# mryndzionek/composable-sdr

Hardware: AMD Instinct MI355X
Metric: MS/s CF32 throughput, 256-ch PFB+FM pipeline (higher is better)
Workload: dtype f32; 1 GPU; cfg3: 256-ch firpfbch(m=7,As=80)+dcBlocker+freqdem(kf=0.3) on synthetic CF32, AGC off (-a 0), 262144 frames/step (512 MiB in, 256 MiB out), HBM-resident; channels=256, demod=fm, mix=False, route=fused-256|k_tile256<FM>, preheat_steps=10999, collective=none, rccl_ranks=1

## Files before the change

composable_sdr_amd/csrc/fused.h:

```cpp
#pragma once
#include "csdr_internal.h"

namespace csdr {

struct FusedConfig {
    uint32_t M, p, C, c0, max_nf;
    uint32_t G = 1;
    bool dc_block; DcParams dc;
    bool fm; float fm_ref;
    bool mix;
    const float *taps;
    uint32_t d_theta;
    uint32_t cus = 256;
};

struct FusedCall {
    const float2 *d_in;
    void *d_out;
    uint32_t nf;
    uint32_t theta0;
    bool indep = false;
    hipEvent_t ev_tail = nullptr;
    bool tile_major = false;
};
// ... 25 lines not shown
    std::vector<float2> premix_table() const;
    virtual int reset_state(hipStream_t s) = 0;
    virtual int run(const FusedCall &call, void *out, hipStream_t s, KernelTimer *timer) = 0;
};

template <class Plan> int make_plan(const FusedConfig &cfg, ChainPlan **out)
{
    Plan *p = new Plan(cfg);
    if (int r = p->init()) { delete p; return r; }
    *out = p;
    return 0;
}

bool plan256_supported(uint32_t M, uint32_t p);
int  plan256_create(const FusedConfig &cfg, ChainPlan **out);
bool plan64_supported(uint32_t M, uint32_t p);
int  plan64_create(const FusedConfig &cfg, ChainPlan **out);
bool plan1024_supported(uint32_t M, uint32_t p);
int  plan1024_create(const FusedConfig &cfg, ChainPlan **out);
bool plan4096_supported(uint32_t M, uint32_t p);
int  plan4096_create(const FusedConfig &cfg, ChainPlan **out);

int  run256_v2_launch(const void *run_args, bool fm, unsigned G, unsigned nruns, hipStream_t s);
int  run256_v2_blocks_per_cu(bool fm);
int  run256_dcfix_launch(const void *run_args, bool fm, unsigned nruns, const float2 *Rt, hipStream_t s);
int  run256_v3_launch(const void *run_args, bool fm, unsigned nruns, hipStream_t s);


struct Run64v2Host {
    const float2 *x; float2 *out;
    const float *taps; const float2 *tw, *wpre;
    const float2 *uhist_in; float2 *uhist_out; const float2 *vend_in; float2 *vend_out;
    float2 *cpre = nullptr; const float2 *rt = nullptr;
    uint32_t nf, nruns, parity0;
    uint32_t G = 1, g = 0;
    bool tile_major = false;
    bool dc_block;
    double beta;
};
constexpr int RUN64_DCFIX_F = 448;
uint32_t run64_v2_runs(uint32_t nf, uint32_t cus);
void dc_state_response(const FusedConfig &cfg, const float2 *wpre, uint32_t f0, uint32_t nfr, uint32_t k0, float2 *rt);
int run64_v2_launch(const Run64v2Host &h, hipStream_t s, KernelTimer *timer);

struct Run1024v2Host {
    const float2 *x; void *out;
    const float4 *taps_q;
// ... 37 lines not shown
```

composable_sdr_amd/csrc/fused_v2_common.h:

```cpp
#pragma once
#include "fused_common.h"

namespace csdr {
namespace {

typedef float v4f __attribute__((ext_vector_type(4)));
#ifndef V2_DMA_AUX
#define V2_DMA_AUX ""
#endif
#ifndef V2_DMA_AUX_STREAM
#define V2_DMA_AUX_STREAM V2_DMA_AUX
#endif

__device__ __forceinline__ void bar()
{
    asm volatile("s_waitcnt lgkmcnt(0)\n\ts_barrier" ::: "memory");
}
__device__ __forceinline__ float opaque_v(float x) { asm volatile("" : "+v"(x)); return x; }

__device__ __forceinline__ unsigned dma_offset(int tid)
{
    const int wave = tid >> 6, lane = tid & 63;
    const int slot = 64 * wave + lane, q = slot >> 3, i = (slot & 7) ^ ((q >> 1) & 7);
    return (unsigned)(8 * q + i) * 16u;
// ... 2 lines not shown
{
    const int wave = tid >> 6, lane = tid & 63;
    const int slot = 64 * wave + lane, q = slot >> 3, i = (slot & 7) ^ (q & 7);
    return (unsigned)(8 * q + i) * 16u;
}
template <bool STREAM = false, unsigned IT_STEP = 4096u>
__device__ __forceinline__ void dma_tile(const float4 *__restrict__ tile_base, unsigned goff, unsigned lds_wave)
{
    asm volatile("" : "+s"(lds_wave));
#pragma unroll
    for (int it = 0; it < 8; it++) {
        const unsigned dst = lds_wave + IT_STEP * (unsigned)it;
        const float4 *src = tile_base + 256 * it;
        unsigned keep;
        if (STREAM)
            asm volatile("s_mov_b32 %0, m0\n\ts_mov_b32 m0, %2\n\ts_nop 4\n\tglobal_load_lds_dwordx4 %1, %3" V2_DMA_AUX_STREAM "\n\ts_mov_b32 m0, %0"
                         : "=&s"(keep) : "v"(goff), "s"(dst), "s"(src) : "memory");
        else
            asm volatile("s_mov_b32 %0, m0\n\ts_mov_b32 m0, %2\n\ts_nop 4\n\tglobal_load_lds_dwordx4 %1, %3" V2_DMA_AUX "\n\ts_mov_b32 m0, %0"
                         : "=&s"(keep) : "v"(goff), "s"(dst), "s"(src) : "memory");
    }
}

__device__ __forceinline__ void dma_piece(const float4 *__restrict__ tile_base, unsigned goff, unsigned lds_wave, const int it)
{
    asm volatile("" : "+s"(lds_wave));
    const unsigned dst = lds_wave + 4096u * (unsigned)it;
    const float4 *src = tile_base + 256 * it;
    unsigned keep;
    asm volatile("s_mov_b32 %0, m0\n\ts_mov_b32 m0, %2\n\ts_nop 4\n\tglobal_load_lds_dwordx4 %1, %3" V2_DMA_AUX "\n\ts_mov_b32 m0, %0"
                 : "=&s"(keep) : "v"(goff), "s"(dst), "s"(src) : "memory");
}

struct FmK { float tiny, ref, hp, pi; };
__device__ __forceinline__ float fm_sample(float2 rp, float2 r, const FmK &k)
{
    const float re = fmaf(rp.x, r.x, rp.y * r.y);
    const float im = fmaf(rp.x, r.y, -(rp.y * r.x));
    const float mx = fmaxf(fmaxf(fabsf(re), fabsf(im)), k.tiny);
    const float mn = fminf(fabsf(re), fabsf(im));
    const float a = mn * __builtin_amdgcn_rcpf(mx);
    const float z = a * a;
    float p = -4.054457881e-03f;
    p = fmaf(p, z, 2.186254039e-02f);
    p = fmaf(p, z, -5.591168255e-02f);
    p = fmaf(p, z, 9.642146528e-02f);
    p = fmaf(p, z, -1.390860826e-01f);
    p = fmaf(p, z, 1.994656026e-01f);
    p = fmaf(p, z, -3.332985938e-01f);
    p = fmaf(p, z, 9.999993443e-01f);
// ... 92 lines not shown
```

composable_sdr_amd/csrc/kernels_fused.hip:

```cpp
#include "fused_common.h"
#include <cstring>

namespace csdr {

namespace {

#define STAMP(i) do { if (A.trace && tid == 0) A.trace[(size_t)b * 16 + (i)] = __builtin_amdgcn_s_memtime(); } while (0)

template <bool FM>
__global__ __launch_bounds__(256) void k_tile256(TileArgs A)
{
    __shared__ __attribute__((aligned(16))) float2 R[LDS_F2];
    __shared__ float2 tw_s[M256];
    __shared__ float2 Tt[2][16];
    __shared__ float2 carry_s[2];
    __shared__ unsigned tile_s;

    const int tid = threadIdx.x;
    if (tid == 0) tile_s = atomicAdd(A.ticket, 1u);
    tw_s[tid] = A.tw[tid];
    __syncthreads();
    const unsigned b = tile_s;
    if (b >= A.nb) return;
    STAMP(0);
// ... 425 lines not shown
    CSDR_HIP(hipMemcpy(d_wpre, wpre.data(), sizeof(float2) * 2 * cfg.M, hipMemcpyHostToDevice));
    if (nowu) {
        std::vector<float2> rt((size_t)2 * DCFIX_F * 4);
        dc_state_response(cfg, wpre.data(), 15u, (uint32_t)DCFIX_F, 126u, rt.data());
        CSDR_HIP(hipMemcpy(d_rt, rt.data(), sizeof(float2) * rt.size(), hipMemcpyHostToDevice));
    }
    CSDR_HIP(hipMemset(d_status, 0, sizeof(unsigned)));
    CSDR_HIP(hipMemset(d_yflag, 0, sizeof(unsigned) * max_nb));
    CSDR_HIP(hipMemset(d_agg, 0, sizeof(u64) * 2 * max_nb));

    TileArgs &A = proto;
    A = TileArgs{};
    A.taps = d_taps; A.tw = d_tw; A.wpre = d_wpre;
    A.ticket = d_ticket; A.agg = d_agg; A.ylast = d_ylast; A.yflag = d_yflag; A.status = d_status;
    A.c0 = cfg.c0; A.C = cfg.C; A.fm_ref = cfg.fm_ref; A.trace = d_trace;
    const double beta = cfg.dc_block ? (double)cfg.dc.beta : 0.0;
    A.alpha = cfg.dc_block ? (float)(1.0 - beta) : 0.0f;
    A.beta = (float)beta;
    for (int k = 0; k < LOOKBACK + 2; k++) A.wtile[k] = (float)std::pow(beta, 4096.0 * k);
    for (int k = 0; k < 16; k++) A.b16[k] = (float)std::pow(beta, 16.0 * k);
    for (int k = 0; k < 17; k++) A.b256[k] = (float)std::pow(beta, 256.0 * k);
    for (int k = 0; k < 16; k++) A.bj[k] = (float)std::pow(beta, (double)k);
    if (const char *e = diag_env("CSDR_CUS")) { if (atoi(e) > 0 && (uint32_t)atoi(e) < cus) cus = (uint32_t)atoi(e); }
    resident_wgs_v2 = (uint32_t)(cus * run256_v2_blocks_per_cu(cfg.fm));
    if (const char *e = diag_env("CSDR_RESIDENT_WGS")) resident_wgs_v2 = (uint32_t)atol(e);
#ifdef CSDR_WITH_RUN256_V3
    if (const char *e = diag_env("CSDR_RUN_V3")) use_v3 = atoi(e) != 0;
#endif
    if (const char *e = diag_env("CSDR_RUN_WEIGHTS")) {
        int k = 0;
        for (const char *q = e; *q && k < 8; k++) { slot_weight[k] = (float)atof(q); q = strchr(q, ','); if (!q) break; q++; }
    }
    return 0;
}

int FusedPlan::reset_state(hipStream_t s)
{
    for (int i = 0; i < 2; i++) {
        CSDR_HIP(hipMemsetAsync(d_yhist[i], 0, sizeof(float2) * 13 * cfg.M, s));
        CSDR_HIP(hipMemsetAsync(d_vend[i], 0, sizeof(float2), s));
        CSDR_HIP(hipMemsetAsync(d_rp[i], 0, sizeof(float2) * (cfg.G > 1 ? cfg.M : cfg.C), s));
    }
    CSDR_HIP(hipMemsetAsync(d_tail[0], 0, sizeof(float4) * 2048 * (WU + 1), s));
    tail_w = 0; tail_valid = true;
    return 0;
}

// ... 22 lines not shown
    A.rp_in = d_rp[cur];       A.rp_out = d_rp[cur ^ 1];
    A.out_stride = nf; A.out_t0 = 0;
    if (call.tile_major) A.out_stride = NB;
    A.parity0 = (uint32_t)(frames_done & 1);
    const uint32_t nb_full = nf / NB;
    const bool shard = c.G > 1;
    if (shard && (uint64_t)c.C * nf * (c.fm ? 4u : 8u) >= (1ull << 32)) { set_error("fused: interleaved shard output of %u frames exceeds 4 GiB", nf); return -1; }
    const bool whole_band = c.G == 1 && c.c0 == 0 && c.C == c.M;
    if ((nb_full >= run_min_tiles && whole_band) || shard) {
        const bool v2 = true;
        const bool v3 = !shard && use_v3;
        kernel = v3 ? (c.fm ? "k_run256v3<FM>" : "k_run256v3<CF32>") : (c.fm ? "k_run256v2<FM>" : "k_run256v2<CF32>");
        if (shard) kernel += "/G" + std::to_string(c.G);
        RunArgs RA{};
        A.nf = nb_full * NB; A.nb = nb_full;
        RA.t = A; RA.pk = phase_consts(c.fm_ref);
        uint32_t nruns = v3 ? cus : resident_wgs_v2;
        if (v3) { if (const char *e = diag_env("CSDR_V3_RUNS")) nruns = (uint32_t)atol(e); }
        if (nruns > A.nb / 8) nruns = A.nb / 8;
        if (nruns < 1) nruns = 1;
        RA.nruns = nruns;
        static const float v2_weight_cf[8] = {1.2f, 0.8f, 1.f, 1.f, 1.f, 1.f, 1.f, 1.f};
        static const float v2_weight_fm[8] = {1.24f, 0.76f, 1.f, 1.f, 1.f, 1.f, 1.f, 1.f};
        const float *v2_weight = c.fm ? v2_weight_fm : v2_weight_cf;
        static const float equal_weight[8] = {1.f, 1.f, 1.f, 1.f, 1.f, 1.f, 1.f, 1.f};
        static const bool pd_equal = diag_env("CSDR_PD_EQUAL") != nullptr;
        RA.split = make_split(A.nb, nruns, cus, (call.indep && pd_equal) ? equal_weight : ((v2 && !diag_env("CSDR_RUN_WEIGHTS")) ? v2_weight : slot_weight));
        { const char *e = diag_env("CSDR_PRIO_ROT"); RA.prio_div = e ? (atoi(e) ? cus : 0u) : (v2 ? 0u : cus); }
        { const char *e = diag_env("CSDR_TRACE"); RA.trace_light = (e && atoi(e) == 2) ? 1u : 0u; }
        { const char *e = diag_env("CSDR_WU"); RA.wu = e ? (uint32_t)atoi(e) : (uint32_t)WU; }
        { const char *e = diag_env("CSDR_WU_ROT"); RA.wu_rot = e ? (uint32_t)atoi(e) : 0u; }
        RA.pair_align = (v2 && (c.fm || diag_env("CSDR_PAIR_ALIGN_CF"))) ? 1u : 0u;
        { const char *e = diag_env("CSDR_WU_BATCH6"); RA.wu_batch6 = e ? (uint32_t)atoi(e) : 1u; }
        RA.l2beta = c.dc_block ? (float)std::log2((double)c.dc.beta) : -1000.0f;
        RA.tile_step = call.tile_major ? c.C * 128u : (uint32_t)NB * (c.fm ? 4u : 8u);
        const bool whole = nf == nb_full * NB;
        RA.indep = call.indep ? 1u : 0u;
        RA.nowu = (nowu && !shard && !v3 && !RA.indep && nruns >= 2 && nruns <= 2048) ? 1u : 0u;
        RA.cpre = d_cpre; RA.side = d_side;
        RA.prev_tail = d_tail[tail_w];
        if (save_tails && !shard && v2 && whole && nb_full >= WU + 1) {
            const int nxt = (tail_w + 1) % 3;
            static const bool nocopy = diag_env("CSDR_PD_NOCOPY") != nullptr;
            if (!nocopy) hipLaunchKernelGGL(k_save_tail, dim3(2048 * (WU + 1) / 256), dim3(256), 0, s,
                                            reinterpret_cast<const float4 *>(call.d_in + (size_t)(nb_full - (WU + 1)) * 4096), d_tail[nxt]);
            if (call.ev_tail) CSDR_HIP(hipEventRecord(call.ev_tail, s));
            tail_w = nxt; tail_valid = true;
// ... 61 lines not shown
```

composable_sdr_amd/csrc/kernels_fused_v2.hip:

```cpp
#ifndef V2_FM_PACKED
#define V2_FM_PACKED 1
#endif
#ifndef V2_ABLATE
#define V2_ABLATE 0
#endif

#ifndef V2_COLSCAN
#define V2_COLSCAN 0
#endif
#ifndef V2_PAIR
#define V2_PAIR 1
#endif
#ifndef V2_STORE_AUX
#define V2_STORE_AUX ""
#endif
#ifndef V2_PAIR_CF
#define V2_PAIR_CF 0
#endif
#ifndef V2_BAR_E
#define V2_BAR_E 0
#endif
#ifndef V2_PAD
#define V2_PAD 1
#endif
#ifndef V2_SNOP
#define V2_SNOP ""
#endif

#include "fused_v2_common.h"
#include <cstddef>
#include <type_traits>

namespace csdr {
namespace {

constexpr unsigned V2_FSB = 2048u + (V2_PAD ? 128u : 0u);
constexpr int V2_FS2 = (int)V2_FSB / 8;
constexpr int V2_BUF = 16 * V2_FS2;
constexpr int V2_STASH = 2 * V2_BUF;
constexpr int V2_F2 = V2_STASH + 256 + 32 + 256 + (V2_COLSCAN ? 512 : 0);
#define V2_ZSW(f) (V2_PAD ? (((f) >> 1) & 7) : ((f) & 7))
#ifndef V2_RSWN
#define V2_RSWN V2_PAD
#endif
#define V2_RSW(a) (V2_RSWN ? ((a) & 7) : (((a) >> 1) & 7))

struct V2Args {
    RunArgs r;
};

template <bool FM, int G>
__global__ __launch_bounds__(256, 2) void k_run256v2(V2Args VA)
{
    static_assert(G == 1 || G == 2 || G == 4 || G == 8, "interleaved shards: G = 2, 4, 8");
    constexpr int NK1 = 16 / G;
    const RunArgs &RA = VA.r;
    const TileArgs &A = RA.t;
    __shared__ __attribute__((aligned(16))) float2 L[V2_F2];
    float2 *R = L, *ST = L + V2_STASH, *Tt = ST + 256, *red = Tt + 16;
    float2 *tw_s = red + 16;
    float2 *TRc = tw_s + 256, *Ec = TRc + 256;
    (void)TRc; (void)Ec;
    float2 *H = L + V2_BUF;
    float2 *E = ST;
    const int tid = threadIdx.x, j = tid;
    const unsigned w = blockIdx.x;
    unsigned first, last;
    run_range(RA.split, w, first, last);
    if (RA.pair_align) {
        first &= ~1u;
        if (last != A.nb) last &= ~1u;
    }
    const float4 *x4 = reinterpret_cast<const float4 *>(A.x);
    const int col_off = 16 * (j >> 4) + 2 * (((j & 15) >> 1) ^ V2_RSW(j >> 4)) + (j & 1);
    const unsigned goff = V2_RSWN ? dma_offset_rsw(tid) : dma_offset(tid);
    const unsigned wave_u = (unsigned)__builtin_amdgcn_readfirstlane(tid >> 6);
    const unsigned lds_wave = (unsigned)(size_t)(__attribute__((address_space(3))) float2 *)R + V2_FSB * (wave_u >> 1) + 1024u * (wave_u & 1u);

#ifndef V2_TRACE
#define V2_TRACE 0
#endif
#if V2_TRACE
#define V2LSTAMP(i) do { if (A.trace && RA.trace_light && tid == 0) A.trace[(size_t)first * 16 + (i)] = __builtin_amdgcn_s_memrealtime(); } while (0)
#else
#define V2LSTAMP(i) do { } while (0)
#endif
    V2LSTAMP(0);
    const bool cold = w > 0 || RA.indep;
    const int halo = (int)first - 1;
    auto tile_ptr = [&](int t) -> const float4 * { return t >= 0 ? x4 + (size_t)t * 2048 : RA.prev_tail + (size_t)(WU + 1 + t) * 2048; };
    if (first < last) dma_tile<false, 2 * V2_FSB>(x4 + (size_t)first * 2048, goff, lds_wave);
    if (cold) dma_tile<false, 2 * V2_FSB>(tile_ptr(halo), goff, lds_wave + (unsigned)(V2_BUF * 8));
    float h[P];
#pragma unroll
    for (int n = 0; n < P; n++) h[n] = A.taps[(M256 - 1 - j) + n * M256];
    float2 Wa = A.wpre[(A.parity0 & 1) * M256 + j], Wb = A.wpre[((A.parity0 & 1) ^ 1) * M256 + j];
    if (G > 1) {
        const int n = ((j >> 4) * (int)A.c0) & 15;
        const float C1 = 0.92387953251128674f, S1 = 0.38268343236508977f, R2 = 0.70710678118654752f;
        const int m4 = n & 3, qd = n >> 2;
        const float2 e = m4 == 0 ? make_float2(1.f, 0.f) : (m4 == 1 ? make_float2(C1, -S1) : (m4 == 2 ? make_float2(R2, -R2) : make_float2(S1, -C1)));
        const float2 rot = qd == 0 ? e : (qd == 1 ? make_float2(e.y, -e.x) : (qd == 2 ? make_float2(-e.x, -e.y) : make_float2(-e.y, e.x)));
        Wa = cmul(Wa, rot); Wb = cmul(Wb, rot);
    }
    tw_s[tid] = A.tw[tid];
    float2 wa[NB], wb[NB];
#pragma unroll
    for (int f = 0; f < NB; f++) { wa[f] = make_float2(0.f, 0.f); wb[f] = make_float2(0.f, 0.f); }
    float2 c;
    float2 w2 = make_float2(0.f, 0.f);

    if (!cold) {
        c = A.vend_in[0];
#pragma unroll
        for (int f = 3; f < NB; f++) wa[f] = A.yhist_in[(f - 3) * M256 + j];
// ... 5 lines not shown
        {
            const int wave = tid >> 6, lane = tid & 63;
            const int slot = 64 * wave + lane, q = slot >> 3;
            const int i = (slot & 7) ^ ((q >> 1) & 7);
            const int n = 16 * q + 2 * i;
            wt0 = exp2f((float)(4095 - n) * RA.l2beta);
            wt1 = exp2f((float)(4094 - n) * RA.l2beta);
        }
        const float wstep = RA.l2beta < -100.0f ? 0.0f : exp2f(-512.0f * RA.l2beta);
        float2 acc = make_float2(0.f, 0.f);
        auto fold = [&](const float4 (&r)[8], int t) {
            float2 p = make_float2(0.f, 0.f);
            float a0 = wt0, a1 = wt1;
#pragma unroll
            for (int it = 0; it < 8; it++) {
                p = cfma(make_float2(r[it].x, r[it].y), a0, p);
                p = cfma(make_float2(r[it].z, r[it].w), a1, p);
                a0 *= wstep; a1 *= wstep;
            }
            acc = cfma(p, exp2f((float)(4096 * (halo - 1 - t)) * RA.l2beta), acc);
        };
        const unsigned rot = RA.wu_rot ? w : 0u;
        unsigned i = 0;
        if (nwu == 6 && RA.wu_batch6) {
            float4 rb[8], rc[8], rd[8], re[8], rf[8];
            const int t0 = h0 + (int)(rot % 6u), t1 = h0 + (int)((1 + rot) % 6u), t2 = h0 + (int)((2 + rot) % 6u);
            const int t3 = h0 + (int)((3 + rot) % 6u), t4 = h0 + (int)((4 + rot) % 6u), t5 = h0 + (int)((5 + rot) % 6u);
            tile_load(tile_ptr(t0), 256, raw, tid); tile_load(tile_ptr(t1), 256, rb, tid); tile_load(tile_ptr(t2), 256, rc, tid);
            tile_load(tile_ptr(t3), 256, rd, tid); tile_load(tile_ptr(t4), 256, re, tid); tile_load(tile_ptr(t5), 256, rf, tid);
            fold(raw, t0); fold(rb, t1); fold(rc, t2); fold(rd, t3); fold(re, t4); fold(rf, t5);
            i = 6;
        } else if (nwu >= 3) {
            float4 rb[8], rc[8];
#pragma unroll 1
            for (; i + 3 <= nwu; i += 3) {
                const int t0 = h0 + (int)((i + rot) % nwu), t1 = h0 + (int)((i + 1 + rot) % nwu), t2 = h0 + (int)((i + 2 + rot) % nwu);
                tile_load(tile_ptr(t0), 256, raw, tid);
                tile_load(tile_ptr(t1), 256, rb, tid);
                tile_load(tile_ptr(t2), 256, rc, tid);
                fold(raw, t0); fold(rb, t1); fold(rc, t2);
            }
        }
        for (; i < nwu; i++) {
            const int t0 = h0 + (int)((i + rot) % nwu);
            tile_load(tile_ptr(t0), 256, raw, tid);
            fold(raw, t0);
        }
        float2 ch = wg_sum(acc, red, tid);
        V2LSTAMP(1);
        if (h0 == 0 && !RA.indep) ch = cfma(A.vend_in[0], exp2f((float)(4096 * halo) * RA.l2beta), ch);
        asm volatile("s_waitcnt vmcnt(0)" ::: "memory");
        __syncthreads();
        scan_staged_fs<V2_FS2, V2_RSWN != 0>(H, E, Tt, A, tid);
#pragma unroll
        for (int f = 3; f < NB; f++) wa[f] = H[V2_FS2 * f + col_off];
        w2 = H[V2_FS2 * 2 + col_off];
        const float kj = -A.alpha * A.bj[j & 15];
        const float br = A.b16[tid & 15], bf = A.b256[tid >> 4];
        float2 vb, ve;
        frame_carries(Tt, A, tid, vb, ve);
        E[tid] = cfma(cfma(ch, bf, vb), br, E[tid]);
        c = cfma(ch, A.b256[16], ve);
        __syncthreads();
#pragma unroll
        for (int f = 3; f < NB; f++) wa[f] = cfma(E[16 * f + (j >> 4)], kj, wa[f]);
        w2 = cfma(E[16 * 2 + (j >> 4)], kj, w2);
    }
#pragma unroll
    for (int f = 3; f < NB; f++) wa[f] = cmul(wa[f], (f & 1) ? Wb : Wa);
    __syncthreads();
    const int st_i = XIDX(tid >> 4), st_j1 = ((tid & 15) - (int)(G > 1 ? A.c0 : 0u)) / G;
    const bool st_own = G == 1 || ((((tid & 15) - (int)A.c0) & (G - 1)) == 0 && (tid & 15) >= (int)A.c0);
    const int st_idx = G == 1 ? (tid & 15) * 16 + st_i : (st_own ? ((st_i / NK1) * NK1 + st_j1) * 16 + st_i : 0);
    if (st_own) ST[st_idx] = (FM && !cold) ? A.rp_in[tid] : make_float2(0.f, 0.f);
    __syncthreads();
    if (FM && cold) {
        w2 = cmul(w2, Wa);
        v2f acc = {0.f, 0.f};
#pragma unroll
        for (int n = P - 1; n >= 0; n--) {
            const float2 s2 = (n == P - 1) ? w2 : wa[NB - 1 - n];
            acc = __builtin_elementwise_fma((v2f){s2.x, s2.y}, (v2f){h[n], h[n]}, acc);
        }
        H[j] = to_f2(acc);
        __syncthreads();
        v2f vv[16];
        if (tid < 16) {
#pragma unroll
            for (int a = 0; a < 16; a++) vv[a] = to_v(H[16 * a + tid]);
            fft16_v(vv);
#pragma unroll
            for (int i = (G > 1 ? 0 : 1); i < 16; i++) vv[i] = cmul_v(vv[i], to_v(tw_s[16 * ((XIDX(i) + (G > 1 ? (int)A.c0 : 0)) & 15) + tid]));
#pragma unroll
            for (int i = 0; i < 16; i++) H[256 + 16 * XIDX(i) + tid] = to_f2(vv[i]);
        }
        __syncthreads();
        if (tid < 16) {
#pragma unroll
            for (int b = 0; b < 16; b++) vv[b] = to_v(H[256 + 16 * (G * (tid % NK1)) + b]);
            fft16_v(vv);
#pragma unroll
            for (int i = 0; i < 16; i++) ST[tid * 16 + i] = to_f2(vv[i]);
            if (G == 1 && RA.nowu) {
                if (tid >= 14) RA.side[((size_t)w * 4 + (tid - 14)) * DCFIX_F] = to_f2(vv[13]);
                else if (tid <= 1) RA.side[((size_t)w * 4 + 2 + tid) * DCFIX_F] = to_f2(vv[2]);
            }
        }
        __syncthreads();
    }

    const v2f Wav = to_v(Wa), Wbv = to_v(Wb);
    const float na = opaque_v(-A.alpha), be = opaque_v(A.beta);
    const float kJ = -A.alpha * exp2f((float)j * RA.l2beta);
    const float b256 = A.b256[1];
    const FmK2 fk = {{opaque_v(9.999993443e-01f), opaque_v(-3.332985938e-01f), opaque_v(1.994656026e-01f), opaque_v(-1.390860826e-01f),
                      opaque_v(9.642146528e-02f), opaque_v(-5.591168255e-02f), opaque_v(2.186254039e-02f), opaque_v(-4.054457881e-03f)},
                     opaque_v(1e-37f), opaque_v(A.fm_ref), opaque_v(RA.pk.hp), opaque_v(RA.pk.pi)};
    const int q = tid, sw = V2_RSW(q & 15);
    const unsigned raw_a = (unsigned)q * 128u + (unsigned)(q >> 4) * (V2_FSB - 2048u) + ((unsigned)sw << 4);
    const int f1 = tid >> 4, b1 = tid & 15;
    const int k1 = tid >> 4, f2 = tid & 15;
    const unsigned x_a = (unsigned)f1 * V2_FSB + (unsigned)b1 * 8u;
    const unsigned zw_a = (unsigned)f1 * V2_FSB + (unsigned)((((b1 >> 1) ^ V2_ZSW(f1)) << 1) | (b1 & 1)) * 8u;
    const unsigned z_a = (unsigned)f2 * V2_FSB + (unsigned)k1 * 128u + ((unsigned)V2_ZSW(f2) << 4);
    const int j1 = k1 % NK1, hb = (G == 8) ? ((k1 >> 1) & 1) : 0;
    const unsigned z_a_g = (unsigned)f2 * V2_FSB + (unsigned)(G * j1) * 128u + ((unsigned)V2_ZSW(f2) << 4);
    const uint32_t voff = ((uint32_t)(G == 1 ? k1 : j1 + 16 * hb) * A.out_stride + A.out_t0 + (uint32_t)f2) * (FM ? 4u : 8u);
    const size_t row16 = (size_t)NK1 * A.out_stride * (FM ? 4u : 8u);
#if V2_TRACE
#define V2STAMP(i) do { if (A.trace && !RA.trace_light && tid == 0) A.trace[(size_t)b_ * 16 + (i)] = __builtin_amdgcn_s_memtime(); } while (0)
#else
#define V2STAMP(i) do { } while (0)
#endif

    float hold[16];
    v2f holdc[V2_PAIR_CF ? 16 : 1];
    auto tile = [&](float2 (&old)[NB], float2 (&nw)[NB], unsigned b_, const int par) {
        unsigned b = (unsigned)__builtin_amdgcn_readfirstlane((int)b_);
        asm volatile("" : "+s"(b));
        char *B = reinterpret_cast<char *>(L) + par * (V2_BUF * 8);
        float2 *Bf = reinterpret_cast<float2 *>(B);
        if (RA.prio_div) {
            if (((b_ - first) + w / RA.prio_div) & 1u) __builtin_amdgcn_s_setprio(1); else __builtin_amdgcn_s_setprio(0);
        }
        V2STAMP(0);
        if (G == 1 && b + 1 == last && tid == 0) {
            if (kernarg_u32_s<offsetof(V2Args, r.nowu)>()) kernarg_ptr_s<offsetof(V2Args, r.cpre)>()[w + 1] = c;
        }
        if (V2_TRACE && A.trace && !RA.trace_light && tid == 0) A.trace[(size_t)b_ * 16 + 15] = __builtin_amdgcn_s_memrealtime();
        bar();
        V2STAMP(1);
#ifdef V2_SELECTIVE_POLICY
        if (!(V2_ABLATE & 1) && b + 1 < last) {
            if (b + 1 + (WU + 1) < last) dma_tile<true, 2 * V2_FSB>(x4 + (size_t)(b + 1) * 2048, goff, lds_wave + (unsigned)(par ^ 1) * (V2_BUF * 8u));
            else dma_tile<false, 2 * V2_FSB>(x4 + (size_t)(b + 1) * 2048, goff, lds_wave + (unsigned)(par ^ 1) * (V2_BUF * 8u));
        }
#else
        if (!(V2_ABLATE & 1) && b + 1 < last) dma_tile<false, 2 * V2_FSB>(x4 + (size_t)(b + 1) * 2048, goff, lds_wave + (unsigned)(par ^ 1) * (V2_BUF * 8u));
#endif
#if V2_COLSCAN
#pragma unroll
        for (int f = 0; f < NB; f++) nw[f] = Bf[V2_FS2 * f + col_off];
        col_run_scan(nw, TRc, A, tid);
        V2STAMP(2);
        bar();
        col_run_carries(TRc, Ec, Tt, A, tid);
        bar();
        V2STAMP(3);
        {
            v2f V = to_v(c);
            const float kj = -A.alpha * A.bj[j & 15];
            const v2f kJv = {kJ, kJ}, bv = {b256, b256}, kjv = {kj, kj};
#pragma unroll
            for (int f = 0; f < NB; f++) {
                v2f y = __builtin_elementwise_fma(V, kJv, to_v(nw[f]));
                nw[f] = to_f2(__builtin_elementwise_fma(to_v(Ec[16 * f + (j >> 4)]), kjv, y));
                V = __builtin_elementwise_fma(V, bv, to_v(Tt[f]));
            }
            c = to_f2(V);
        }
#else
        v4f xr[8];
        float2 s = make_float2(0.f, 0.f);
#pragma unroll
        for (int i = 0; i < 8; i++) {
            xr[i] = *reinterpret_cast<const v4f *>(B + (raw_a ^ (unsigned)(i << 4)));
            if (V2_ABLATE & 32) { s.x += xr[i].x; continue; }
            s = make_float2(fmaf(s.x, be, xr[i].x), fmaf(s.y, be, xr[i].y));
            s = make_float2(fmaf(s.x, be, xr[i].z), fmaf(s.y, be, xr[i].w));
        }
        {
            float2 t;
            t = dpp2<0x111>(s); s = cfma(t, A.b16[1], s);
            t = dpp2<0x112>(s); s = cfma(t, A.b16[2], s);
            t = dpp2<0x114>(s); s = cfma(t, A.b16[4], s);
            t = dpp2<0x118>(s); s = cfma(t, A.b16[8], s);
        }
        if ((q & 15) == 15) Tt[q >> 4] = s;
        s = dpp2<0x111>(s);
#pragma unroll
        for (int i = 0; i < 8; i++) {
            v4f y;
            if (V2_ABLATE & 32) { *reinterpret_cast<v4f *>(B + (raw_a ^ (unsigned)(i << 4))) = xr[i]; continue; }
            y.x = fmaf(s.x, na, xr[i].x); y.y = fmaf(s.y, na, xr[i].y);
            s = make_float2(fmaf(s.x, be, xr[i].x), fmaf(s.y, be, xr[i].y));
            y.z = fmaf(s.x, na, xr[i].z); y.w = fmaf(s.y, na, xr[i].w);
            s = make_float2(fmaf(s.x, be, xr[i].z), fmaf(s.y, be, xr[i].w));
            if (V2_ABLATE & 64) asm volatile("" :: "v"(y));
            else *reinterpret_cast<v4f *>(B + (raw_a ^ (unsigned)(i << 4))) = y;
        }
        V2STAMP(2);
        bar();
        V2STAMP(3);
#pragma unroll
        for (int f = 0; f < NB; f++) nw[f] = Bf[V2_FS2 * f + col_off];
        {
            v2f V = to_v(c);
            const v2f kJv = {kJ, kJ}, bv = {b256, b256};
#pragma unroll
            for (int f = 0; f < NB; f++) {
                nw[f] = to_f2(__builtin_elementwise_fma(V, kJv, to_v(nw[f])));
                V = __builtin_elementwise_fma(V, bv, to_v(Tt[f]));
            }
            c = to_f2(V);
        }
#endif
        if (b + 1 == A.nb) {
#pragma unroll
            for (int f = 3; f < NB; f++) A.yhist_out[(f - 3) * M256 + j] = nw[f];
        }
#pragma unroll
        for (int f = 0; f < NB; f += 2) {
            v2f a0 = to_v(nw[f]), a1 = to_v(nw[f + 1]);
            cmul2_v(a0, Wav, a1, Wbv);
            nw[f] = to_f2(a0); nw[f + 1] = to_f2(a1);
        }
        V2STAMP(4);
#pragma unroll
        for (int f0 = 0; f0 < NB; f0 += 4) {
            v2f acc[4] = {{0.f, 0.f}, {0.f, 0.f}, {0.f, 0.f}, {0.f, 0.f}};
#pragma unroll
            for (int n = ((V2_ABLATE & 8) ? 0 : P - 1); n >= 0; n--) {
#pragma unroll
                for (int u = 0; u < 4; u++) {
                    const int i = f0 + u - n;
                    const float2 s2 = (i >= 0) ? nw[i] : old[NB + i];
                    const v2f sv = {s2.x, s2.y}, hv = {h[n], h[n]};
                    acc[u] = __builtin_elementwise_fma(sv, hv, acc[u]);
                }
            }
#pragma unroll
            for (int u = 0; u < 4; u++) Bf[V2_FS2 * (f0 + u) + col_off] = to_f2(acc[u]);
        }
        V2STAMP(5);
        bar();
        V2STAMP(6);
        v2f vv[16];
#pragma unroll
        for (int a = 0; a < 16; a++) vv[a] = to_v(*reinterpret_cast<const float2 *>(B + (x_a ^ (unsigned)(V2_RSW(a) << 4)) + 128 * a));
        if (!(V2_ABLATE & 16)) fft16_v(vv);
        if (G == 1) {
#pragma unroll
            for (int i = 1; i < 16; i++) vv[i] = cmul_v(vv[i], to_v(tw_s[16 * XIDX(i) + b1]));
        } else {
#pragma unroll
            for (int i = 0; i < 16; i++)
                if (XIDX(i) % G == 0) vv[i] = cmul_v(vv[i], to_v(tw_s[16 * ((XIDX(i) + (int)A.c0) & 15) + b1]));
        }
        V2STAMP(7);
        if (V2_BAR_E) bar();
        V2STAMP(8);
#pragma unroll
        for (int i = 0; i < 16; i++) {
            if (V2_ABLATE & 128) { asm volatile("" :: "v"(vv[i])); continue; }
            if (XIDX(i) % G == 0) *reinterpret_cast<float2 *>(B + zw_a + 128 * XIDX(i)) = to_f2(vv[i]);
        }
        V2STAMP(9);
        bar();
        V2STAMP(10);
        if constexpr (G > 1) {
// ... 51 lines not shown
                    }
                    if (f2 == 15) {
#pragma unroll
                        for (int u = 0; u < NS; u += 2) *reinterpret_cast<v4f *>(stp + u) = (v4f){y[u].x, y[u].y, y[u + 1].x, y[u + 1].y};
                    }
                } else {
#pragma unroll
                    for (int u = 0; u < NS; u++) {
                        const char *rowp = obase + (size_t)XIDX(S0 + u) * row16;
                        asm volatile("s_nop 4\n\tglobal_store_dwordx2 %0, %1, %2\n\ts_nop 1" :: "v"(voff), "v"(y[u]), "s"(rowp) : "memory");
                    }
                }
            };
            if (G == 2) { if (wave_u < 2u) shard_tail(std::integral_constant<int, 0>{}); else shard_tail(std::integral_constant<int, 2>{}); }
            else switch (wave_u) {
                case 0: shard_tail(std::integral_constant<int, 0>{}); break;
                case 1: shard_tail(std::integral_constant<int, 1>{}); break;
                case 2: shard_tail(std::integral_constant<int, 2>{}); break;
                default: shard_tail(std::integral_constant<int, 3>{}); break;
            }
            V2STAMP(14);
            return;
        }
#pragma unroll
        for (int i = 0; i < 8; i++) {
            const v4f v = *reinterpret_cast<const v4f *>(B + (z_a ^ (unsigned)(i << 4)));
            vv[2 * i] = (v2f){v.x, v.y}; vv[2 * i + 1] = (v2f){v.z, v.w};
        }
        if (!(V2_ABLATE & 16)) fft16_v(vv);
        V2STAMP(11);
        if (G == 1 && cold && b - first < 7u && kernarg_u32_s<offsetof(V2Args, r.nowu)>()) {
            float2 *sd = kernarg_ptr_s<offsetof(V2Args, r.side)>() + ((size_t)w * 4) * DCFIX_F + 1 + 16 * (size_t)(b - first) + f2;
            if (k1 >= 14) sd[(k1 - 14) * DCFIX_F] = to_f2(vv[13]);
            else if (k1 <= 1) sd[(2 + k1) * DCFIX_F] = to_f2(vv[2]);
        }
        char *obase = reinterpret_cast<char *>(A.out) + (size_t)b * RA.tile_step;
        if (FM) {
            asm volatile("s_waitcnt vmcnt(0)" ::: "memory");
#pragma unroll
            for (int i = 0; i < 16; i += 4) {
                float2 rp[4], rr[4];
#pragma unroll
                for (int u = 0; u < 4; u += 2) {
                    const v4f sp = *reinterpret_cast<const v4f *>(ST + k1 * 16 + i + u);
                    rp[u] = make_float2(dpp_keep<0x111>(sp.x, vv[i + u].x), dpp_keep<0x111>(sp.y, vv[i + u].y));
                    rp[u + 1] = make_float2(dpp_keep<0x111>(sp.z, vv[i + u + 1].x), dpp_keep<0x111>(sp.w, vv[i + u + 1].y));
                    rr[u] = to_f2(vv[i + u]); rr[u + 1] = to_f2(vv[i + u + 1]);
                }
                float mq_[4];
                float (&mq)[4] = (V2_PAIR && par == 0) ? *reinterpret_cast<float (*)[4]>(&hold[i]) : mq_;
                if (V2_ABLATE & 4) { mq[0] = rp[0].x + rr[0].y; mq[1] = rp[1].y + rr[1].x; mq[2] = rp[2].x + rr[2].y; mq[3] = rp[3].y + rr[3].x; }
                else if (V2_FM_PACKED) fm_quad(rp, rr, fk, mq);
                else {
                    const FmK k1s = {fk.tiny, fk.ref, fk.hp, fk.pi};
#pragma unroll
                    for (int u = 0; u < 4; u++) mq[u] = fm_sample(rp[u], rr[u], k1s);
                }
                if (V2_PAIR && par == 0 && b + 1 < last) continue;
#pragma unroll
                for (int u = 0; u < 4; u++) {
                    const char *rowp = obase + (size_t)XIDX(i + u) * row16;
                    if (V2_ABLATE & 2) asm volatile("" :: "v"(mq[u]), "s"(rowp));
                    else {
                        if (V2_PAIR && par == 1) asm volatile(V2_SNOP "global_store_dword %0, %1, %2 offset:-64" V2_STORE_AUX :: "v"(voff), "v"(hold[i + u]), "s"(rowp) : "memory");
                        asm volatile(V2_SNOP "global_store_dword %0, %1, %2" V2_STORE_AUX :: "v"(voff), "v"(mq[u]), "s"(rowp) : "memory");
                    }
                }
            }
            if (f2 == 15) {
#pragma unroll
                for (int i = 0; i < 16; i += 2) *reinterpret_cast<v4f *>(ST + k1 * 16 + i) = (v4f){vv[i].x, vv[i].y, vv[i + 1].x, vv[i + 1].y};
            }
            V2STAMP(12);
            V2STAMP(13);
        } else {
            V2STAMP(12);
            asm volatile("s_waitcnt vmcnt(0)" ::: "memory");
            V2STAMP(13);
            if (V2_PAIR_CF && par == 0 && b + 1 < last) {
#pragma unroll
                for (int i = 0; i < 16; i++) holdc[i] = vv[i];
            } else {
#pragma unroll
                for (int i = 0; i < 16; i++) {
                    const char *rowp = obase + (size_t)XIDX(i) * row16;
                    if (V2_ABLATE & 2) asm volatile("" :: "v"(vv[i]), "s"(rowp));
                    else {
                        if (V2_PAIR_CF && par == 1) asm volatile(V2_SNOP "global_store_dwordx2 %0, %1, %2 offset:-128" V2_STORE_AUX :: "v"(voff), "v"(holdc[i]), "s"(rowp) : "memory");
                        asm volatile(V2_SNOP "global_store_dwordx2 %0, %1, %2" V2_STORE_AUX :: "v"(voff), "v"(vv[i]), "s"(rowp) : "memory");
                    }
                }
            }
        }
        V2STAMP(14);
// ... 66 lines not shown
    return 0;
}

static V2Args make_v2(const void *run_args)
{
    V2Args VA;
    VA.r = *static_cast<const RunArgs *>(run_args);
    return VA;
}

int run256_v2_launch(const void *run_args, bool fm, unsigned G, unsigned nruns, hipStream_t s)
{
    const V2Args VA = make_v2(run_args);
#define V2_LAUNCH(F, GG) hipLaunchKernelGGL((k_run256v2<F, GG>), dim3(nruns), dim3(256), 0, s, VA)
    if (G == 1) { if (fm) V2_LAUNCH(true, 1); else V2_LAUNCH(false, 1); }
    else if (G == 2) { if (fm) V2_LAUNCH(true, 2); else V2_LAUNCH(false, 2); }
    else if (G == 4) { if (fm) V2_LAUNCH(true, 4); else V2_LAUNCH(false, 4); }
    else if (G == 8) { if (fm) V2_LAUNCH(true, 8); else V2_LAUNCH(false, 8); }
    else { set_error("k_run256v2: interleaved shards of stride %u are not built (2, 4, 8)", G); return -1; }
#undef V2_LAUNCH
    return 0;
}

int run256_v2_blocks_per_cu(bool fm)
{
    int occ = 0;
    if (fm) (void)hipOccupancyMaxActiveBlocksPerMultiprocessor(&occ, (k_run256v2<true, 1>), 256, 0);
    else (void)hipOccupancyMaxActiveBlocksPerMultiprocessor(&occ, (k_run256v2<false, 1>), 256, 0);
    return occ < 1 ? 1 : occ;
}

}
```

Baseline: 297,600 MS/s.

## Single-buffer FM 256-ch kernel to fit three workgroups per CU

For the FM, G=1 path, the kernel drops the double-buffered LDS input tile in favour of a single buffer. It keeps filter taps in LDS instead of registers to cut VGPR pressure, and raises launch bounds to three workgroups per CU. The next tile's DMA is issued in pieces after the current tile's LDS reads finish, with partial vmcnt waits, so the prefetch still overlaps the FFT and FM work. Run-split weights are retuned for the three-runs-per-CU case. The risks are less overlap from the single buffer, extra LDS traffic for taps, and possible register spills under the tighter bound.

New measurement: 312,100 MS/s, median of 6. 1.05x the previous value.

```diff
diff --git a/composable_sdr_amd/csrc/fused.h b/composable_sdr_amd/csrc/fused.h
--- a/composable_sdr_amd/csrc/fused.h
+++ b/composable_sdr_amd/csrc/fused.h
@@ -71,7 +71,7 @@
 int  plan4096_create(const FusedConfig &cfg, ChainPlan **out);
 
 int  run256_v2_launch(const void *run_args, bool fm, unsigned G, unsigned nruns, hipStream_t s);
-int  run256_v2_blocks_per_cu(bool fm);
+int  run256_v2_blocks_per_cu(bool fm, unsigned G);
 int  run256_dcfix_launch(const void *run_args, bool fm, unsigned nruns, const float2 *Rt, hipStream_t s);
 int  run256_v3_launch(const void *run_args, bool fm, unsigned nruns, hipStream_t s);
 
diff --git a/composable_sdr_amd/csrc/fused_v2_common.h b/composable_sdr_amd/csrc/fused_v2_common.h
--- a/composable_sdr_amd/csrc/fused_v2_common.h
+++ b/composable_sdr_amd/csrc/fused_v2_common.h
@@ -48,10 +48,11 @@
     }
 }
 
+template <unsigned IT_STEP = 4096u>
 __device__ __forceinline__ void dma_piece(const float4 *__restrict__ tile_base, unsigned goff, unsigned lds_wave, const int it)
 {
     asm volatile("" : "+s"(lds_wave));
-    const unsigned dst = lds_wave + 4096u * (unsigned)it;
+    const unsigned dst = lds_wave + IT_STEP * (unsigned)it;
     const float4 *src = tile_base + 256 * it;
     unsigned keep;
     asm volatile("s_mov_b32 %0, m0\n\ts_mov_b32 m0, %2\n\ts_nop 4\n\tglobal_load_lds_dwordx4 %1, %3" V2_DMA_AUX "\n\ts_mov_b32 m0, %0"
diff --git a/composable_sdr_amd/csrc/kernels_fused.hip b/composable_sdr_amd/csrc/kernels_fused.hip
--- a/composable_sdr_amd/csrc/kernels_fused.hip
+++ b/composable_sdr_amd/csrc/kernels_fused.hip
@@ -471,7 +471,7 @@
     for (int k = 0; k < 17; k++) A.b256[k] = (float)std::pow(beta, 256.0 * k);
     for (int k = 0; k < 16; k++) A.bj[k] = (float)std::pow(beta, (double)k);
     if (const char *e = diag_env("CSDR_CUS")) { if (atoi(e) > 0 && (uint32_t)atoi(e) < cus) cus = (uint32_t)atoi(e); }
-    resident_wgs_v2 = (uint32_t)(cus * run256_v2_blocks_per_cu(cfg.fm));
+    resident_wgs_v2 = (uint32_t)(cus * run256_v2_blocks_per_cu(cfg.fm, cfg.G));
     if (const char *e = diag_env("CSDR_RESIDENT_WGS")) resident_wgs_v2 = (uint32_t)atol(e);
 #ifdef CSDR_WITH_RUN256_V3
     if (const char *e = diag_env("CSDR_RUN_V3")) use_v3 = atoi(e) != 0;
@@ -540,7 +540,8 @@
         RA.nruns = nruns;
         static const float v2_weight_cf[8] = {1.2f, 0.8f, 1.f, 1.f, 1.f, 1.f, 1.f, 1.f};
         static const float v2_weight_fm[8] = {1.24f, 0.76f, 1.f, 1.f, 1.f, 1.f, 1.f, 1.f};
-        const float *v2_weight = c.fm ? v2_weight_fm : v2_weight_cf;
+        static const float v2_weight_fm3[8] = {1.45f, 1.f, 0.55f, 1.f, 1.f, 1.f, 1.f, 1.f};
+        const float *v2_weight = c.fm ? ((cus && nruns == 3 * cus) ? v2_weight_fm3 : v2_weight_fm) : v2_weight_cf;
         static const float equal_weight[8] = {1.f, 1.f, 1.f, 1.f, 1.f, 1.f, 1.f, 1.f};
         static const bool pd_equal = diag_env("CSDR_PD_EQUAL") != nullptr;
         RA.split = make_split(A.nb, nruns, cus, (call.indep && pd_equal) ? equal_weight : ((v2 && !diag_env("CSDR_RUN_WEIGHTS")) ? v2_weight : slot_weight));
diff --git a/composable_sdr_amd/csrc/kernels_fused_v2.hip b/composable_sdr_amd/csrc/kernels_fused_v2.hip
--- a/composable_sdr_amd/csrc/kernels_fused_v2.hip
+++ b/composable_sdr_amd/csrc/kernels_fused_v2.hip
@@ -22,6 +22,12 @@
 #endif
 #ifndef V2_PAD
 #define V2_PAD 1
+#endif
+#ifndef V2_ONE_WGS
+#define V2_ONE_WGS 3
+#endif
+#ifndef V2_ONE_BURST
+#define V2_ONE_BURST 1
 #endif
 #ifndef V2_SNOP
 #define V2_SNOP ""
@@ -38,7 +44,9 @@
 constexpr int V2_FS2 = (int)V2_FSB / 8;
 constexpr int V2_BUF = 16 * V2_FS2;
 constexpr int V2_STASH = 2 * V2_BUF;
-constexpr int V2_F2 = V2_STASH + 256 + 32 + 256 + (V2_COLSCAN ? 512 : 0);
+constexpr int V2_AUX2 = 256 + 32 + 256 + (V2_COLSCAN ? 512 : 0);
+constexpr int V2_F2 = V2_STASH + V2_AUX2;
+constexpr int V2_F2_ONE = V2_BUF + V2_AUX2 + P * M256 / 2;
 #define V2_ZSW(f) (V2_PAD ? (((f) >> 1) & 7) : ((f) & 7))
 #ifndef V2_RSWN
 #define V2_RSWN V2_PAD
@@ -50,18 +58,21 @@
 };
 
 template <bool FM, int G>
-__global__ __launch_bounds__(256, 2) void k_run256v2(V2Args VA)
+__global__ __launch_bounds__(256, (FM && G == 1) ? V2_ONE_WGS : 2) void k_run256v2(V2Args VA)
 {
     static_assert(G == 1 || G == 2 || G == 4 || G == 8, "interleaved shards: G = 2, 4, 8");
     constexpr int NK1 = 16 / G;
+    constexpr bool ONE = FM && G == 1;
     const RunArgs &RA = VA.r;
     const TileArgs &A = RA.t;
-    __shared__ __attribute__((aligned(16))) float2 L[V2_F2];
-    float2 *R = L, *ST = L + V2_STASH, *Tt = ST + 256, *red = Tt + 16;
+    __shared__ __attribute__((aligned(16))) float2 L[(ONE && V2_ONE_WGS >= 3) ? V2_F2_ONE : V2_F2];
+    float2 *R = L, *ST = L + (ONE ? V2_BUF : V2_STASH), *Tt = ST + 256, *red = Tt + 16;
     float2 *tw_s = red + 16;
     float2 *TRc = tw_s + 256, *Ec = TRc + 256;
     (void)TRc; (void)Ec;
-    float2 *H = L + V2_BUF;
+    float *TP = reinterpret_cast<float *>(L + (ONE ? V2_BUF : V2_STASH) + V2_AUX2);
+    float2 *H = ONE ? L : L + V2_BUF;
+    float2 *HS = ONE ? reinterpret_cast<float2 *>(TP) : H;
     float2 *E = ST;
     const int tid = threadIdx.x, j = tid;
     const unsigned w = blockIdx.x;
@@ -89,8 +100,13 @@
     const bool cold = w > 0 || RA.indep;
     const int halo = (int)first - 1;
     auto tile_ptr = [&](int t) -> const float4 * { return t >= 0 ? x4 + (size_t)t * 2048 : RA.prev_tail + (size_t)(WU + 1 + t) * 2048; };
-    if (first < last) dma_tile<false, 2 * V2_FSB>(x4 + (size_t)first * 2048, goff, lds_wave);
-    if (cold) dma_tile<false, 2 * V2_FSB>(tile_ptr(halo), goff, lds_wave + (unsigned)(V2_BUF * 8));
+    if (ONE) {
+        if (cold) dma_tile<false, 2 * V2_FSB>(tile_ptr(halo), goff, lds_wave);
+        else if (first < last) dma_tile<false, 2 * V2_FSB>(x4 + (size_t)first * 2048, goff, lds_wave);
+    } else {
+        if (first < last) dma_tile<false, 2 * V2_FSB>(x4 + (size_t)first * 2048, goff, lds_wave);
+        if (cold) dma_tile<false, 2 * V2_FSB>(tile_ptr(halo), goff, lds_wave + (unsigned)(V2_BUF * 8));
+    }
     float h[P];
 #pragma unroll
     for (int n = 0; n < P; n++) h[n] = A.taps[(M256 - 1 - j) + n * M256];
@@ -142,7 +158,7 @@
         };
         const unsigned rot = RA.wu_rot ? w : 0u;
         unsigned i = 0;
-        if (nwu == 6 && RA.wu_batch6) {
+        if (!ONE && nwu == 6 && RA.wu_batch6) {
             float4 rb[8], rc[8], rd[8], re[8], rf[8];
             const int t0 = h0 + (int)(rot % 6u), t1 = h0 + (int)((1 + rot) % 6u), t2 = h0 + (int)((2 + rot) % 6u);
             const int t3 = h0 + (int)((3 + rot) % 6u), t4 = h0 + (int)((4 + rot) % 6u), t5 = h0 + (int)((5 + rot) % 6u);
@@ -182,6 +198,7 @@
         E[tid] = cfma(cfma(ch, bf, vb), br, E[tid]);
         c = cfma(ch, A.b256[16], ve);
         __syncthreads();
+        if (ONE && first < last) dma_tile<false, 2 * V2_FSB>(x4 + (size_t)first * 2048, goff, lds_wave);
 #pragma unroll
         for (int f = 3; f < NB; f++) wa[f] = cfma(E[16 * f + (j >> 4)], kj, wa[f]);
         w2 = cfma(E[16 * 2 + (j >> 4)], kj, w2);
@@ -202,22 +219,22 @@
             const float2 s2 = (n == P - 1) ? w2 : wa[NB - 1 - n];
             acc = __builtin_elementwise_fma((v2f){s2.x, s2.y}, (v2f){h[n], h[n]}, acc);
         }
-        H[j] = to_f2(acc);
+        HS[j] = to_f2(acc);
         __syncthreads();
         v2f vv[16];
         if (tid < 16) {
 #pragma unroll
-            for (int a = 0; a < 16; a++) vv[a] = to_v(H[16 * a + tid]);
+            for (int a = 0; a < 16; a++) vv[a] = to_v(HS[16 * a + tid]);
             fft16_v(vv);
 #pragma unroll
             for (int i = (G > 1 ? 0 : 1); i < 16; i++) vv[i] = cmul_v(vv[i], to_v(tw_s[16 * ((XIDX(i) + (G > 1 ? (int)A.c0 : 0)) & 15) + tid]));
 #pragma unroll
-            for (int i = 0; i < 16; i++) H[256 + 16 * XIDX(i) + tid] = to_f2(vv[i]);
+            for (int i = 0; i < 16; i++) HS[256 + 16 * XIDX(i) + tid] = to_f2(vv[i]);
         }
         __syncthreads();
         if (tid < 16) {
 #pragma unroll
-            for (int b = 0; b < 16; b++) vv[b] = to_v(H[256 + 16 * (G * (tid % NK1)) + b]);
+            for (int b = 0; b < 16; b++) vv[b] = to_v(HS[256 + 16 * (G * (tid % NK1)) + b]);
             fft16_v(vv);
 #pragma unroll
             for (int i = 0; i < 16; i++) ST[tid * 16 + i] = to_f2(vv[i]);
@@ -229,6 +246,10 @@
         __syncthreads();
     }
 
+    if (ONE) {
+#pragma unroll
+        for (int n = 0; n < P; n++) TP[M256 * n + j] = h[n];
+    }
     const v2f Wav = to_v(Wa), Wbv = to_v(Wb);
     const float na = opaque_v(-A.alpha), be = opaque_v(A.beta);
     const float kJ = -A.alpha * exp2f((float)j * RA.l2beta);
@@ -237,12 +258,12 @@
                       opaque_v(9.642146528e-02f), opaque_v(-5.591168255e-02f), opaque_v(2.186254039e-02f), opaque_v(-4.054457881e-03f)},
                      opaque_v(1e-37f), opaque_v(A.fm_ref), opaque_v(RA.pk.hp), opaque_v(RA.pk.pi)};
     const int q = tid, sw = V2_RSW(q & 15);
-    const unsigned raw_a = (unsigned)q * 128u + (unsigned)(q >> 4) * (V2_FSB - 2048u) + ((unsigned)sw << 4);
+    const unsigned raw_a_ = (unsigned)q * 128u + (unsigned)(q >> 4) * (V2_FSB - 2048u) + ((unsigned)sw << 4);
     const int f1 = tid >> 4, b1 = tid & 15;
     const int k1 = tid >> 4, f2 = tid & 15;
-    const unsigned x_a = (unsigned)f1 * V2_FSB + (unsigned)b1 * 8u;
+    const unsigned x_a_ = (unsigned)f1 * V2_FSB + (unsigned)b1 * 8u;
     const unsigned zw_a = (unsigned)f1 * V2_FSB + (unsigned)((((b1 >> 1) ^ V2_ZSW(f1)) << 1) | (b1 & 1)) * 8u;
-    const unsigned z_a = (unsigned)f2 * V2_FSB + (unsigned)k1 * 128u + ((unsigned)V2_ZSW(f2) << 4);
+    const unsigned z_a_ = (unsigned)f2 * V2_FSB + (unsigned)k1 * 128u + ((unsigned)V2_ZSW(f2) << 4);
     const int j1 = k1 % NK1, hb = (G == 8) ? ((k1 >> 1) & 1) : 0;
     const unsigned z_a_g = (unsigned)f2 * V2_FSB + (unsigned)(G * j1) * 128u + ((unsigned)V2_ZSW(f2) << 4);
     const uint32_t voff = ((uint32_t)(G == 1 ? k1 : j1 + 16 * hb) * A.out_stride + A.out_t0 + (uint32_t)f2) * (FM ? 4u : 8u);
@@ -258,11 +279,13 @@
     auto tile = [&](float2 (&old)[NB], float2 (&nw)[NB], unsigned b_, const int par) {
         unsigned b = (unsigned)__builtin_amdgcn_readfirstlane((int)b_);
         asm volatile("" : "+s"(b));
-        char *B = reinterpret_cast<char *>(L) + par * (V2_BUF * 8);
+        char *B = reinterpret_cast<char *>(L) + (ONE ? 0 : par) * (V2_BUF * 8);
         float2 *Bf = reinterpret_cast<float2 *>(B);
         if (RA.prio_div) {
             if (((b_ - first) + w / RA.prio_div) & 1u) __builtin_amdgcn_s_setprio(1); else __builtin_amdgcn_s_setprio(0);
         }
+        int tid_t = tid;
+        if (ONE) asm volatile("" : "+v"(tid_t));
         V2STAMP(0);
         if (G == 1 && b + 1 == last && tid == 0) {
             if (kernarg_u32_s<offsetof(V2Args, r.nowu)>()) kernarg_ptr_s<offsetof(V2Args, r.cpre)>()[w + 1] = c;
@@ -276,8 +299,14 @@
             else dma_tile<false, 2 * V2_FSB>(x4 + (size_t)(b + 1) * 2048, goff, lds_wave + (unsigned)(par ^ 1) * (V2_BUF * 8u));
         }
 #else
-        if (!(V2_ABLATE & 1) && b + 1 < last) dma_tile<false, 2 * V2_FSB>(x4 + (size_t)(b + 1) * 2048, goff, lds_wave + (unsigned)(par ^ 1) * (V2_BUF * 8u));
-#endif
+        if (!ONE && !(V2_ABLATE & 1) && b + 1 < last) dma_tile<false, 2 * V2_FSB>(x4 + (size_t)(b + 1) * 2048, goff, lds_wave + (unsigned)(par ^ 1) * (V2_BUF * 8u));
+#endif
+        auto next_pieces = [&](const int it) {
+            if (ONE && !(V2_ABLATE & 1) && b + 1 < last) {
+                dma_piece<2 * V2_FSB>(x4 + (size_t)(b + 1) * 2048, goff, lds_wave, it);
+                dma_piece<2 * V2_FSB>(x4 + (size_t)(b + 1) * 2048, goff, lds_wave, it + 1);
+            }
+        };
 #if V2_COLSCAN
 #pragma unroll
         for (int f = 0; f < NB; f++) nw[f] = Bf[V2_FS2 * f + col_off];
@@ -302,6 +331,7 @@
 #else
         v4f xr[8];
         float2 s = make_float2(0.f, 0.f);
+        const unsigned raw_a = ONE ? (unsigned)tid_t * 128u + (unsigned)(tid_t >> 4) * (V2_FSB - 2048u) + ((unsigned)V2_RSW(tid_t & 15) << 4) : raw_a_;
 #pragma unroll
         for (int i = 0; i < 8; i++) {
             xr[i] = *reinterpret_cast<const v4f *>(B + (raw_a ^ (unsigned)(i << 4)));
@@ -316,7 +346,7 @@
             t = dpp2<0x114>(s); s = cfma(t, A.b16[4], s);
             t = dpp2<0x118>(s); s = cfma(t, A.b16[8], s);
         }
-        if ((q & 15) == 15) Tt[q >> 4] = s;
+        if (((ONE ? tid_t : q) & 15) == 15) Tt[(ONE ? tid_t : q) >> 4] = s;
         s = dpp2<0x111>(s);
 #pragma unroll
         for (int i = 0; i < 8; i++) {
@@ -346,8 +376,9 @@
         }
 #endif
         if (b + 1 == A.nb) {
-#pragma unroll
-            for (int f = 3; f < NB; f++) A.yhist_out[(f - 3) * M256 + j] = nw[f];
+            float2 *yo = (ONE ? kernarg_ptr_s<offsetof(V2Args, r.t.yhist_out)>() : A.yhist_out) + (ONE ? tid_t : j);
+#pragma unroll
+            for (int f = 3; f < NB; f++) yo[(f - 3) * M256] = nw[f];
         }
 #pragma unroll
         for (int f = 0; f < NB; f += 2) {
@@ -356,6 +387,9 @@
             nw[f] = to_f2(a0); nw[f + 1] = to_f2(a1);
         }
         V2STAMP(4);
+        float ht[P];
+#pragma unroll
+        for (int n = 0; n < P; n++) ht[n] = ONE ? TP[M256 * n + j] : h[n];
 #pragma unroll
         for (int f0 = 0; f0 < NB; f0 += 4) {
             v2f acc[4] = {{0.f, 0.f}, {0.f, 0.f}, {0.f, 0.f}, {0.f, 0.f}};
@@ -365,7 +399,7 @@
                 for (int u = 0; u < 4; u++) {
                     const int i = f0 + u - n;
                     const float2 s2 = (i >= 0) ? nw[i] : old[NB + i];
-                    const v2f sv = {s2.x, s2.y}, hv = {h[n], h[n]};
+                    const v2f sv = {s2.x, s2.y}, hv = {ht[n], ht[n]};
                     acc[u] = __builtin_elementwise_fma(sv, hv, acc[u]);
                 }
             }
@@ -376,6 +410,7 @@
         bar();
         V2STAMP(6);
         v2f vv[16];
+        const unsigned x_a = ONE ? (unsigned)(tid_t >> 4) * V2_FSB + (unsigned)(tid_t & 15) * 8u : x_a_;
 #pragma unroll
         for (int a = 0; a < 16; a++) vv[a] = to_v(*reinterpret_cast<const float2 *>(B + (x_a ^ (unsigned)(V2_RSW(a) << 4)) + 128 * a));
         if (!(V2_ABLATE & 16)) fft16_v(vv);
@@ -473,21 +508,28 @@
             V2STAMP(14);
             return;
         }
+        const unsigned z_a = ONE ? (unsigned)(tid_t & 15) * V2_FSB + (unsigned)(tid_t >> 4) * 128u + ((unsigned)V2_ZSW(tid_t & 15) << 4) : z_a_;
 #pragma unroll
         for (int i = 0; i < 8; i++) {
             const v4f v = *reinterpret_cast<const v4f *>(B + (z_a ^ (unsigned)(i << 4)));
             vv[2 * i] = (v2f){v.x, v.y}; vv[2 * i + 1] = (v2f){v.z, v.w};
         }
+        if (ONE) {
+            bar();
+            next_pieces(0);
+            if (V2_ONE_BURST) { next_pieces(2); next_pieces(4); next_pieces(6); }
+        }
         if (!(V2_ABLATE & 16)) fft16_v(vv);
         V2STAMP(11);
         if (G == 1 && cold && b - first < 7u && kernarg_u32_s<offsetof(V2Args, r.nowu)>()) {
-            float2 *sd = kernarg_ptr_s<offsetof(V2Args, r.side)>() + ((size_t)w * 4) * DCFIX_F + 1 + 16 * (size_t)(b - first) + f2;
-            if (k1 >= 14) sd[(k1 - 14) * DCFIX_F] = to_f2(vv[13]);
-            else if (k1 <= 1) sd[(2 + k1) * DCFIX_F] = to_f2(vv[2]);
+            const int k1s = ONE ? tid_t >> 4 : k1, f2s = ONE ? tid_t & 15 : f2;
+            float2 *sd = kernarg_ptr_s<offsetof(V2Args, r.side)>() + ((size_t)w * 4) * DCFIX_F + 1 + 16 * (size_t)(b - first) + f2s;
+            if (k1s >= 14) sd[(k1s - 14) * DCFIX_F] = to_f2(vv[13]);
+            else if (k1s <= 1) sd[(2 + k1s) * DCFIX_F] = to_f2(vv[2]);
         }
         char *obase = reinterpret_cast<char *>(A.out) + (size_t)b * RA.tile_step;
         if (FM) {
-            asm volatile("s_waitcnt vmcnt(0)" ::: "memory");
+            if (!ONE) asm volatile("s_waitcnt vmcnt(0)" ::: "memory");
 #pragma unroll
             for (int i = 0; i < 16; i += 4) {
                 float2 rp[4], rr[4];
@@ -507,6 +549,7 @@
 #pragma unroll
                     for (int u = 0; u < 4; u++) mq[u] = fm_sample(rp[u], rr[u], k1s);
                 }
+                if (!V2_ONE_BURST && i < 12) next_pieces(2 + i / 2);
                 if (V2_PAIR && par == 0 && b + 1 < last) continue;
 #pragma unroll
                 for (int u = 0; u < 4; u++) {
@@ -521,6 +564,10 @@
             if (f2 == 15) {
 #pragma unroll
                 for (int i = 0; i < 16; i += 2) *reinterpret_cast<v4f *>(ST + k1 * 16 + i) = (v4f){vv[i].x, vv[i].y, vv[i + 1].x, vv[i + 1].y};
+            }
+            if (ONE && b + 1 < last) {
+                if ((V2_PAIR && par == 0) || (V2_ABLATE & 2)) asm volatile("s_waitcnt vmcnt(0)" ::: "memory");
+                else asm volatile("s_waitcnt vmcnt(%0)" :: "n"((V2_ONE_BURST ? 4 : 2) * (V2_PAIR ? 8 : 4)) : "memory");
             }
             V2STAMP(12);
             V2STAMP(13);
@@ -633,10 +680,12 @@
     return 0;
 }
 
-int run256_v2_blocks_per_cu(bool fm)
+int run256_v2_blocks_per_cu(bool fm, unsigned G)
 {
     int occ = 0;
-    if (fm) (void)hipOccupancyMaxActiveBlocksPerMultiprocessor(&occ, (k_run256v2<true, 1>), 256, 0);
+    if (G != 1) { if (fm) (void)hipOccupancyMaxActiveBlocksPerMultiprocessor(&occ, (k_run256v2<true, 2>), 256, 0);
+                  else (void)hipOccupancyMaxActiveBlocksPerMultiprocessor(&occ, (k_run256v2<false, 2>), 256, 0); }
+    else if (fm) (void)hipOccupancyMaxActiveBlocksPerMultiprocessor(&occ, (k_run256v2<true, 1>), 256, 0);
     else (void)hipOccupancyMaxActiveBlocksPerMultiprocessor(&occ, (k_run256v2<false, 1>), 256, 0);
     return occ < 1 ? 1 : occ;
 }
```
